# TurakhiaLab/TWILIGHT

Measured on AMD Instinct MI355X. Metric: DP band cells/s, TALCO-XDrop progressive profile-profile alignment (bit-exact vs reference CPU path), higher is better.
Workload: dtype f32

## Files before the change

### include/twl_align.h

```cpp
#ifndef TWL_ALIGN_H
#define TWL_ALIGN_H

#include <stdint.h>

#ifdef __cplusplus
extern "C" {
#endif

#define TWL_MAX_MATRIX 21
#define TWL_MAX_MARKER 1024

enum twl_status {
    TWL_OK = 0,
    TWL_ERR_NOT_INITIALIZED = -1,
    TWL_ERR_BAD_ARGUMENT = -2,
    TWL_ERR_HIP = -3,
    TWL_ERR_UNSUPPORTED = -4
};

typedef struct twl_params {
    int32_t P;
    float   matrix[TWL_MAX_MATRIX * TWL_MAX_MATRIX];
    float   gap_open;
    float   gap_extend;
// ... 43 lines not shown

int twl_copy_to_device(int device, void *dst_dev, const void *src, uint64_t bytes);
int twl_copy_from_device(int device, void *dst, const void *src_dev, uint64_t bytes);
int twl_copy_rows_from_device(int device, void *dst, uint64_t dst_pitch, const void *src_dev, uint64_t src_pitch, uint64_t width, uint64_t rows);

int twl_get_stats(int device, twl_stats *out);

int twl_get_pair_cells(int device, uint64_t *cells_out, int32_t n);

int twl_column_scores(const twl_params *p, int32_t seq_len, const float *freq, const int32_t *len, const int32_t *num, float *out);

int twl_dp_column_scores(const twl_params *p, int32_t seq_len, const float *freq, const float *gap_open, const float *gap_extend,
                         const int32_t *len, const int32_t *num, float *out);

#define TWL_MT_REC_WORDS 12
typedef struct twl_mt_dims {
    int32_t n_run, slots, sp_pitch, segcap;
    int32_t n_scout, n_tile, rounds;
    int32_t lead2, marg, anchors;
    int32_t thr, small_tiles, marker;
    int32_t reserved[3];
} twl_mt_dims;
int twl_mt_tables(int device, twl_mt_dims *dims, int32_t *order, int32_t *anchor, int32_t *spath, int32_t *chain, int32_t *rec, int8_t *seg, int32_t *front);

#define TWL_COMM_ID_BYTES 128
int twl_comm_unique_id(void *id128);
int twl_comm_init(int device, int rank, int world, const void *id128);
int twl_comm_all_gather(int device, const void *d_send, void *d_recv, int64_t bytes_per_rank);
int twl_comm_all_gather_host(int device, const void *send, void *recv, int64_t bytes_per_rank);
int twl_comm_destroy(int device);

enum twl_knob { TWL_KNOB_MT_PERTURB = 1, TWL_KNOB_MT_MAX_PAIRS = 2, TWL_KNOB_MT_MIN_MARKER = 3, TWL_KNOB_MT_LEAD = 4, TWL_KNOB_MT_MARGIN = 5,
                TWL_KNOB_MT_ROUNDS = 6, TWL_KNOB_MT_THR_JOBS = 7, TWL_KNOB_FAIL_ROW_ALLOCS = 8,
                TWL_KNOB_PROT_MODE = 9, TWL_KNOB_ASSUME_ONEHOT_QUERY = 10, TWL_KNOB_MT_TAIL_PCT = 11, TWL_KNOB_MT_WIDE = 12, TWL_KNOB_NO_SPEC = 13, TWL_KNOB_SCOUT_XDROP_PCT = 14, TWL_KNOB_THR_SMALL = 15, TWL_KNOB_FORCE_GLOBAL = 16, TWL_KNOB_LEAF_STEP = 17, TWL_KNOB_POISON_TB = 18, TWL_KNOB_MT_ANCHOR = 19, TWL_KNOB_MT_LEAD2 = 20, TWL_KNOB_PROT_CORRIDOR = 21 };
int twl_set_knob(int key, int value);
int twl_plan_describe(const twl_params *p, int32_t n_pairs, const int32_t *len, int32_t num_cu, int32_t qry_onehot, int32_t wide_streak, char *out, int32_t cap);

#ifdef __cplusplus
}
#endif
#endif
```

### twilight_amd/api.py

```python
from __future__ import annotations

import ctypes as C
import os

import numpy as np

_HERE = os.path.dirname(os.path.abspath(__file__))
LIB_PATH = os.environ.get("TWL_LIB") or os.path.join(_HERE, "libtwl_align.so")
TWL_MAX_MATRIX = 21

_lib = None


class TwlError(RuntimeError):
    pass


class TwlParams(C.Structure):
    _fields_ = [("P", C.c_int32), ("matrix", C.c_float * (TWL_MAX_MATRIX * TWL_MAX_MATRIX)), ("gap_open", C.c_float),
                ("gap_extend", C.c_float), ("gap_boundary", C.c_float), ("gap_char", C.c_float), ("xdrop", C.c_int32),
                ("flen", C.c_int32), ("marker", C.c_int32)]


class TwlStats(C.Structure):
# ... 94 lines not shown
    n, sl = batch.n_pairs, batch.seq_len
    freq = np.ascontiguousarray(batch.freq, dtype=np.float32)
    go = np.ascontiguousarray(batch.gap_open, dtype=np.float32)
    ge = np.ascontiguousarray(batch.gap_extend, dtype=np.float32)
    ln = np.ascontiguousarray(batch.len, dtype=np.int32)
    nm = np.ascontiguousarray(batch.num, dtype=np.int32)
    aln = np.zeros((n, 2 * sl), dtype=np.int8)
    aln_len = np.zeros(n, dtype=np.int32)
    err = np.zeros(n, dtype=np.int16)
    _check(lib.twl_align_batch(C.byref(params), C.c_int32(n), C.c_int32(sl), _ptr(freq, C.c_float), _ptr(go, C.c_float),
                               _ptr(ge, C.c_float), _ptr(ln, C.c_int32), _ptr(nm, C.c_int32), _ptr(aln, C.c_int8),
                               _ptr(aln_len, C.c_int32), _ptr(err, C.c_int16)))
    return aln, aln_len, err


def align_batch_device(params: TwlParams, n_pairs, seq_len, d_freq, d_gop, d_gex, d_len, d_num, d_aln, d_aln_len, d_err,
                       device=0, stream=None):
    lib = load_library()
    vp = C.c_void_p
    _check(lib.twl_align_batch_device(C.c_int(device), vp(stream or 0), C.byref(params), C.c_int32(n_pairs), C.c_int32(seq_len),
                                      vp(d_freq), vp(d_gop), vp(d_gex), vp(d_len), vp(d_num), vp(d_aln), vp(d_aln_len),
                                      vp(d_err)))


KNOB_MT_PERTURB, KNOB_MT_MAX_PAIRS, KNOB_MT_MIN_MARKER, KNOB_MT_LEAD, KNOB_MT_MARGIN, KNOB_MT_ROUNDS, KNOB_MT_THR_JOBS, KNOB_FAIL_ROW_ALLOCS = 1, 2, 3, 4, 5, 6, 7, 8
KNOB_PROT_MODE, KNOB_ASSUME_ONEHOT_QUERY, KNOB_MT_TAIL_PCT, KNOB_MT_WIDE, KNOB_NO_SPEC, KNOB_SCOUT_XDROP_PCT = 9, 10, 11, 12, 13, 14
KNOB_THR_SMALL = 15
KNOB_FORCE_GLOBAL = 16
KNOB_LEAF_STEP = 17
KNOB_POISON_TB = 18
KNOB_MT_ANCHOR = 19
KNOB_PROT_CORRIDOR = 21
KNOB_MT_LEAD2 = 20
PROT_MODES = {"auto": 0, "dense": 1, "sparse": 2, "presim": 3, "r1": 4, "lean_sparse": 5, "lean_presim": 6}


def set_knob(key: int, value: int):
    _check(load_library().twl_set_knob(C.c_int(key), C.c_int(value)))


def plan_describe(params, lens, num_cu=256, qry_onehot=False, wide_streak=0, small_state=0) -> str:
    wide_streak = int(wide_streak) + (100000 * (32 + int(small_state)) if small_state else 0)
    lens = np.ascontiguousarray(lens, dtype=np.int32)
    buf = C.create_string_buffer(256)
    _check(load_library().twl_plan_describe(C.byref(params), C.c_int32(lens.shape[0]), _ptr(lens, C.c_int32), C.c_int32(num_cu), C.c_int32(int(qry_onehot)), C.c_int32(wide_streak), buf, C.c_int32(256)))
    return buf.value.decode()


def version() -> str:
    return load_library().twl_version().decode()


def get_stats(device=0) -> TwlStats:
    st = TwlStats()
    _check(load_library().twl_get_stats(C.c_int(device), C.byref(st)))
    return st


def get_pair_cells(n, device=0):
    out = np.zeros(n, dtype=np.uint64)
    _check(load_library().twl_get_pair_cells(C.c_int(device), _ptr(out, C.c_uint64), C.c_int32(n)))
    return out


def column_scores(params: TwlParams, ref: np.ndarray, qry: np.ndarray, ref_num: int, qry_num: int) -> np.ndarray:
    ref = np.ascontiguousarray(ref, dtype=np.float32)
# ... 44 lines not shown
```

### twilight_amd/csrc/twl_align.hip

```cpp
#include "../../include/twl_align.h"
#include "../../include/twl_level.h"
#include "../../include/twl_place.h"
#include "../../include/twl_merge.h"
#include "../../include/twl_subtree.h"
#include "../../include/twl_guide.h"
#include "../../include/twl_retree.h"
#include "level_kernels.hip.h"
#include "restore_kernels.hip.h"
#include "place_kernels.hip.h"
#include "merge_kernels.hip.h"
#include "subtree_kernels.hip.h"
#include "guide_kernels.hip.h"
#include "retree_kernels.hip.h"
#include "talco_kernel.hip.h"
#include "talco_nuc.hip.h"
#include "talco_global.hip.h"

#include <hip/hip_runtime.h>
#include <dlfcn.h>

#include <algorithm>
#include <atomic>
#include <chrono>
#include <cmath>
// ... 46 lines not shown
#define HIP_TRY(expr)                                                                                          \
    do {                                                                                                       \
        hipError_t e_ = (expr);                                                                                \
        if (e_ != hipSuccess) {                                                                                \
            g_err = std::string(#expr) + ": " + hipGetErrorString(e_);                                         \
            return TWL_ERR_HIP;                                                                                \
        }                                                                                                      \
    } while (0)


#include "twl_policy.inc.hip"

struct Buf {
    void *p = nullptr;
    size_t cap = 0;
    int ensure(size_t bytes)
    {
        if (bytes <= cap) return TWL_OK;
        if (p) (void)hipFree(p);
        p = nullptr; cap = 0;
        size_t want = bytes + bytes / 8 + 256;
        HIP_TRY(hipMalloc(&p, want));
        cap = want;
        return TWL_OK;
    }
    void release() { if (p) (void)hipFree(p); p = nullptr; cap = 0; }
};

struct Device {
    int id = 0;
    hipStream_t stream = nullptr;
    hipStream_t stream2 = nullptr;
    hipEvent_t ev2[2] = {};
    hipEvent_t ev[8] = {};
    int num_cu = 0;
    Buf cols, tb, cells, queue, items, errs, dbg;
    Buf gtb;
    Buf sim, sim_off, blk_off, m24;
    Buf team;
    Buf mt_chain, mt_rec, mt_seg, mt_spath, mt_stat, mt_jobs, mt_anchor;
    Buf simdump;
    bool dump_on = false;
    std::vector<int32_t> dbg_host;
    std::vector<int32_t> mt_jobs_host;
    twl_mt_dims mt_dims{};
    std::vector<int32_t> mt_order;
    bool mt_seen = false;
    Buf gc_zero;
    std::vector<uint8_t> gc_zero_host;
    std::vector<int16_t> last_err;
    void *probe_h = nullptr; size_t probe_cap = 0;
    PassMemory mem;
    int live_stores = 0;
    void *comm = nullptr;
    int comm_world = 0, comm_rank = 0;
    Buf comm_send, comm_recv;
    int mt_launch = 0;
    char kname[160] = {0};
    Buf h2d_freq, h2d_gop, h2d_gex, h2d_len, h2d_num, d_aln, d_alnlen, d_err;
    twl_stats stats{};
    std::vector<uint64_t> pair_cells;
    twl::FillArgs fills{};
    char *res_h = nullptr; size_t res_cap = 0;
    std::vector<int32_t> last_alnlen;
    std::mutex mu;
};
// ... 46 lines not shown
}

static void twl_level_pool_release(Device *d);
namespace { extern int g_fail_next_row_allocs; void comm_destroy_raw(void *comm); }

extern "C" {

const char *twl_last_error(void) { return g_err.c_str(); }
#ifndef TWL_SOURCE_HASH
#define TWL_SOURCE_HASH "unstamped"
#endif
#ifndef TWL_BUILD_STAMP
#define TWL_BUILD_STAMP "unstamped"
#endif
__attribute__((used)) static const char twl_build_stamp[] = "TWLSTAMP:" TWL_BUILD_STAMP ";";
const char *twl_version(void) { return "twilight_amd 0.5 (gfx950) src " TWL_SOURCE_HASH; }

int twl_init(const int *device_ids, int n_devices)
{
    std::lock_guard<std::mutex> lk(g_mu);
    if (g_init) return TWL_OK;
    int count = 0;
    HIP_TRY(hipGetDeviceCount(&count));
    if (count < 1) { g_err = "no HIP device"; return TWL_ERR_HIP; }
    std::vector<int> ids;
    if (!device_ids || n_devices <= 0) ids.push_back(0);
    else ids.assign(device_ids, device_ids + n_devices);
    std::vector<Device *> devs;
    auto fail = [&](int rc) {
        for (auto *d : devs) {
            for (auto &e : d->ev) if (e) (void)hipEventDestroy(e);
            if (d->stream) (void)hipStreamDestroy(d->stream);
            if (d->stream2) (void)hipStreamDestroy(d->stream2);
            for (auto &e : d->ev2) if (e) (void)hipEventDestroy(e);
            delete d;
        }
        return rc;
    };
    for (int id : ids) {
        if (id < 0 || id >= count) { g_err = "device id out of range"; return fail(TWL_ERR_BAD_ARGUMENT); }
        auto *d = new Device();
        d->id = id;
        devs.push_back(d);
        hipDeviceProp_t prop;
        hipError_t e = hipSetDevice(id);
        if (e == hipSuccess) e = hipGetDeviceProperties(&prop, id);
        if (e == hipSuccess) { d->num_cu = prop.multiProcessorCount; e = hipStreamCreateWithFlags(&d->stream, hipStreamNonBlocking); if (e == hipSuccess) { int least = 0, greatest = 0; (void)hipDeviceGetStreamPriorityRange(&least, &greatest); e = hipStreamCreateWithPriority(&d->stream2, hipStreamNonBlocking, least); } }
        for (auto &ev : d->ev2) if (e == hipSuccess) e = hipEventCreate(&ev);
        for (auto &ev : d->ev) if (e == hipSuccess) e = hipEventCreate(&ev);
        if (e != hipSuccess) { g_err = std::string("twl_init: ") + hipGetErrorString(e); return fail(TWL_ERR_HIP); }
    }
    g_devs = devs;
    g_init = true;
#ifdef TWL_DEV
    static const struct { const char *env; int knob; } kEnvKnobs[] = {{"TWL_MT_MAX_PAIRS", TWL_KNOB_MT_MAX_PAIRS}, {"TWL_MT_LEAD", TWL_KNOB_MT_LEAD}, {"TWL_MT_MARGIN", TWL_KNOB_MT_MARGIN},
        {"TWL_MT_PERTURB", TWL_KNOB_MT_PERTURB}, {"TWL_MT_ROUNDS", TWL_KNOB_MT_ROUNDS}, {"TWL_MT_THR_JOBS", TWL_KNOB_MT_THR_JOBS}, {"TWL_MT_TAIL_PCT", TWL_KNOB_MT_TAIL_PCT}};
    for (const auto &k : kEnvKnobs) if (const char *v = getenv(k.env)) (void)twl_set_knob(k.knob, atoi(v));
#endif
    return TWL_OK;
}

void twl_shutdown(void)
{
    std::lock_guard<std::mutex> lk(g_mu);
    for (auto *d : g_devs) {
        std::lock_guard<std::mutex> dl(d->mu);
        if (d->live_stores > 0) {
            fprintf(stderr, "twl_shutdown: %d store(s) still alive on device %d; the library stays initialised (twl_store_destroy them first)\n", d->live_stores, d->id);
            return;
        }
    }
    for (auto *d : g_devs) {
        (void)hipSetDevice(d->id);
        (void)hipStreamSynchronize(d->stream);
        (void)hipStreamSynchronize(d->stream2);
        twl_level_pool_release(d);
        if (d->comm) { comm_destroy_raw(d->comm); d->comm = nullptr; }
        d->comm_send.release(); d->comm_recv.release();
        for (Buf *b : {&d->cols, &d->tb, &d->gtb, &d->cells, &d->queue, &d->items, &d->errs, &d->dbg, &d->sim, &d->sim_off, &d->blk_off, &d->m24, &d->team, &d->simdump, &d->mt_chain, &d->mt_rec, &d->mt_seg, &d->mt_spath, &d->mt_stat, &d->mt_jobs, &d->mt_anchor, &d->gc_zero,
                       &d->h2d_freq, &d->h2d_gop, &d->h2d_gex, &d->h2d_len, &d->h2d_num, &d->d_aln, &d->d_alnlen, &d->d_err})
            b->release();
        for (auto &e : d->ev) if (e) (void)hipEventDestroy(e);
        if (d->stream) (void)hipStreamDestroy(d->stream);
        if (d->stream2) (void)hipStreamDestroy(d->stream2);
        for (auto &e : d->ev2) if (e) (void)hipEventDestroy(e);
        if (d->res_h) (void)hipHostFree(d->res_h);
        if (d->probe_h) (void)hipHostFree(d->probe_h);
        delete d;
    }
    g_devs.clear();
    g_init = false;
}

int twl_align_batch_device(int device, void *stream, const twl_params *p, int32_t n_pairs, int32_t seq_len, const float *d_freq,
                           const float *d_gap_open, const float *d_gap_extend, const int32_t *d_len, const int32_t *d_num,
                           int8_t *d_aln_out, int32_t *d_aln_len_out, int16_t *d_err_out)
{
    if (!g_init) { g_err = "twl_init not called"; return TWL_ERR_NOT_INITIALIZED; }
    int rc = check_params(p);
    if (rc) return rc;
    if (n_pairs < 0 || seq_len < 1) { g_err = "bad n_pairs/seq_len"; return TWL_ERR_BAD_ARGUMENT; }
    Device *d = nullptr;
    if ((rc = find_dev(device, &d))) return rc;
    std::lock_guard<std::mutex> lk(d->mu);
    hipStream_t st = stream ? (hipStream_t)stream : d->stream;
    return run_device(d, st, p, n_pairs, seq_len, d_freq, d_gap_open, d_gap_extend, d_len, d_num, d_aln_out, d_aln_len_out,
                      d_err_out, nullptr);
}

static int run_host_slice(Device *d, const twl_params *p, const std::vector<int32_t> &ids, int32_t seq_len, const float *freq,
                          const float *gop, const float *gex, const int32_t *len, const int32_t *num, int8_t *aln_out,
                          int32_t *aln_len_out, int16_t *err_out)
{
    std::lock_guard<std::mutex> lk(d->mu);
    HIP_TRY(hipSetDevice(d->id));
    const int32_t n = (int32_t)ids.size();
    d->stats = twl_stats{};
    d->pair_cells.clear();
// ... 243 lines not shown
    int rc = find_dev(device, &d);
    if (rc) return rc;
    if (width == 0 || rows == 0) return TWL_OK;
    if (!dst || !src_dev || dst_pitch < width || src_pitch < width) { g_err = "bad argument"; return TWL_ERR_BAD_ARGUMENT; }
    HIP_TRY(hipSetDevice(d->id));
    HIP_TRY(hipMemcpy2D(dst, (size_t)dst_pitch, src_dev, (size_t)src_pitch, (size_t)width, (size_t)rows, hipMemcpyDeviceToHost));
    return TWL_OK;
}

int twl_set_knob(int key, int value)
{
    std::lock_guard<std::mutex> lk(g_mu);
    switch (key) {
    case TWL_KNOB_MT_PERTURB: g_mt_perturb = std::max(0, value); return TWL_OK;
    case TWL_KNOB_MT_MAX_PAIRS: g_mt_max_pairs = std::max(0, value); return TWL_OK;
    case TWL_KNOB_MT_MIN_MARKER: g_mt_min_marker = std::max(2, value); return TWL_OK;
    case TWL_KNOB_MT_LEAD: g_mt_lead = std::max(16, value); return TWL_OK;
    case TWL_KNOB_MT_MARGIN: if (value < 0) { g_mt_marg = 40; g_mt_marg_lat = 64; } else g_mt_marg = g_mt_marg_lat = std::max(2, value); return TWL_OK;
    case TWL_KNOB_MT_ROUNDS: g_mt_rounds = std::max(1, std::min(7, value)); return TWL_OK;
    case TWL_KNOB_MT_THR_JOBS: g_mt_thr_jobs = std::max(0, value); return TWL_OK;
    case TWL_KNOB_FAIL_ROW_ALLOCS: g_fail_next_row_allocs = std::max(0, value); return TWL_OK;
    case TWL_KNOB_PROT_MODE: if (value < 0 || value > 6) { g_err = "protein mode 0..6"; return TWL_ERR_BAD_ARGUMENT; } g_prot_mode = value; return TWL_OK;
    case TWL_KNOB_ASSUME_ONEHOT_QUERY: g_assume_onehot_query = value ? 1 : 0; return TWL_OK;
    case TWL_KNOB_MT_TAIL_PCT: g_mt_tail_pct = std::max(0, std::min(100, value)); return TWL_OK;
    case TWL_KNOB_MT_WIDE: g_mt_wide = value ? 1 : 0; return TWL_OK;
    case TWL_KNOB_NO_SPEC: g_no_spec = value ? 1 : 0; return TWL_OK;
    case TWL_KNOB_FORCE_GLOBAL: g_force_global = value ? 1 : 0; return TWL_OK;
    case TWL_KNOB_LEAF_STEP: g_leaf_step = value ? 1 : 0; return TWL_OK;
    case TWL_KNOB_POISON_TB: g_poison_tb = value ? 1 : 0; return TWL_OK;
    case TWL_KNOB_MT_ANCHOR: g_mt_anchor = value ? 1 : 0; return TWL_OK;
    case TWL_KNOB_MT_LEAD2: if (value < 0) { g_mt_lead2 = 96; g_mt_lead2_lat = 128; } else g_mt_lead2 = g_mt_lead2_lat = std::max(16, value); return TWL_OK;
    case TWL_KNOB_PROT_CORRIDOR: g_prot_corridor = std::max(0, value); for (auto *d : g_devs) d->mem.forget_corridor(); return TWL_OK;
    case TWL_KNOB_SCOUT_XDROP_PCT: g_scout_xdrop_pct = std::max(10, std::min(100, value)); return TWL_OK;
    case TWL_KNOB_THR_SMALL: g_thr_small = std::max(0, std::min(2, value)); for (auto *d : g_devs) d->mem.forget_small(); return TWL_OK;
    default: g_err = "unknown knob"; return TWL_ERR_BAD_ARGUMENT;
    }
}

#include "twl_comm.inc.hip"

int twl_plan_describe(const twl_params *p, int32_t n_pairs, const int32_t *len, int32_t num_cu, int32_t qry_onehot, int32_t wide_streak, char *out, int32_t cap)
{
    if (!p || (p->P != 6 && p->P != 22) || n_pairs < 0 || (n_pairs > 0 && !len) || num_cu < 1 || !out || cap < 64) { g_err = "bad argument (nucleotide or protein parameters, a buffer of 64+ bytes)"; return TWL_ERR_BAD_ARGUMENT; }
    const PassMemory mem = memory_from_code(wide_streak);
    std::vector<int32_t> order;
    for (int32_t n = 0; n < n_pairs; ++n) if (len[2 * n] > 0 && len[2 * n + 1] > 0) order.push_back(n);
    std::stable_sort(order.begin(), order.end(), [&](int32_t x, int32_t y) { return (int64_t)len[2 * x] + len[2 * x + 1] > (int64_t)len[2 * y] + len[2 * y + 1]; });
    const int ms = p->P - 1;
    std::vector<float> M(p->matrix, p->matrix + ms * ms);
    if (p->P == 22) {
        ProtFacts pf;
        pf.n_run = (int)order.size(); pf.n_pairs = n_pairs; pf.num_cu = num_cu; pf.marker = p->marker; pf.M = M.data(); pf.gap_char = p->gap_char;
        pf.corridor_lost = mem.corridor_lost; pf.h_len = len; pf.order = order.data();
        const ProtPlan pl = plan_protein(pf, current_knobs());
        const int w = snprintf(out, (size_t)cap, "%s; mode %d; window %d", prot_first_name(pl.first), pl.mm, prot_first_window(pl.first));
        if (pl.presim && w > 0 && w < cap) snprintf(out + w, (size_t)(cap - w), "; %zu scores precomputed, corridor %d", pl.simFloats, pl.corridor);
        return TWL_OK;
    }
    NucFacts nf;
    nf.n_run = (int)order.size(); nf.num_cu = num_cu; nf.marker = p->marker; nf.M = M.data(); nf.gap_char = p->gap_char; nf.qry_onehot = qry_onehot != 0;
    nf.remember(mem); nf.h_len = len; nf.order = order.data();
    const NucPlan pl = plan_nucleotide(nf, current_knobs());
    snprintf(out, (size_t)cap, "%s; mode %d; window %d%s; bulk %d tail %d", nuc_first_name(pl.first), pl.mm5 ? 5 : pl.mm,
             pl.first == NucFirst::WideMt ? 3072 : ((pl.first == NucFirst::Throughput && pl.small) ? 512 : ((pl.first == NucFirst::Throughput && pl.four) ? 768 : 1024)), pl.probe ? " or 768 (a sample of the level decides)" : "", pl.bulk, pl.tail);
    return TWL_OK;
}
// ... 34 lines not shown
```

### twilight_amd/csrc/twl_knobs.inc.hip

```cpp

int g_prot_corridor = 448;
int g_mt_perturb = 0;
int g_mt_lead = 320, g_mt_marg = 40;
int g_mt_marg_lat = 64, g_mt_lead2_lat = 128;
int g_mt_anchor = 1, g_mt_lead2 = 96;
int g_mt_max_pairs = 1024, g_mt_min_marker = 512, g_mt_rounds = 2, g_mt_thr_jobs = 256;
int g_scout_xdrop_pct = 100;
int g_no_spec = 0;
int g_thr_small = 0;
int g_mt_wide = 1;
int g_mt_tail_pct = 70;
int g_prot_mode = 0;
int g_force_global = 0;
int g_assume_onehot_query = 0;
int g_leaf_step = 1;
int g_poison_tb = 0;
Knobs current_knobs()
{
    return Knobs{g_mt_max_pairs, g_mt_min_marker, g_mt_tail_pct, g_mt_wide, g_assume_onehot_query, g_no_spec, g_thr_small, (ProtMode)g_prot_mode, g_prot_corridor,
                 g_mt_thr_jobs, g_mt_rounds, g_mt_anchor, g_mt_lead, g_mt_marg, g_mt_marg_lat, g_mt_lead2, g_mt_lead2_lat};
}
```

### twilight_amd/csrc/twl_launch.inc.hip

```cpp

template <class CfgT>
size_t tb_words_for(int marker) { return ((size_t)(marker >> 3) + 1) * (size_t)CfgT::WINDOW; }
int ensure_tb(Buf &b, hipStream_t st, size_t words, int grid)
{
    const size_t bytes = words * sizeof(uint32_t) * (size_t)grid;
    if (const int rc = b.ensure(bytes)) return rc;
    if (g_poison_tb) HIP_TRY(hipMemsetAsync(b.p, 0xFF, bytes, st));
    return TWL_OK;
}
template <auto Kernel, int THREADS>
int resident_per_cu(int *out)
{
    static std::atomic<int> cached{0};
    if (cached.load() == 0) {
        int nb = 0;
        HIP_TRY(hipOccupancyMaxActiveBlocksPerMultiprocessor(&nb, Kernel, THREADS, 0));
        cached.store(std::max(1, nb));
    }
    *out = cached.load();
    return TWL_OK;
}
twl::NArgs lean_args(const Device *d, const twl::KArgs &base)
{
    twl::NArgs a{};
// ... 82 lines not shown
}

template <int P, int W, int RPL, int MM, int MINW, bool SPEC = false, bool DUMP = false, int SP = 0>
int launch_lean(Device *d, hipStream_t st, const twl::KArgs &base, const int32_t *d_items, int n_items, int *grid_out, int *window_out)
{
    using CfgT = twl::NCfg<W, RPL>;
    int rc, blocks_per_cu = 0;
    if ((rc = resident_per_cu<twl::talco_lean_kernel<P, W, RPL, MM, MINW, SPEC, DUMP, 0, SP>, CfgT::THREADS>(&blocks_per_cu))) return rc;
    if (window_out) *window_out = CfgT::WINDOW;
    int grid = std::min(n_items, d->num_cu * blocks_per_cu);
    if (grid < 1) grid = 1;
    if (SPEC) {
        grid = 2 * n_items;
        if (grid > d->num_cu * blocks_per_cu) { g_err = "speculative launch larger than the device"; return TWL_ERR_BAD_ARGUMENT; }
    }
    const size_t tbw = tb_words_for<CfgT>(base.marker);
    if ((rc = ensure_tb(d->tb, st, tbw, grid))) return rc;
    twl::NArgs a = lean_args(d, base);
    a.tb = (uint32_t *)d->tb.p; a.tb_words = (int32_t)tbw; a.queue = base.queue; a.items = d_items; a.n_items = n_items; a.dbg = base.dbg;
    FILL_TRY(queue_fill(d, st, d->queue.p, sizeof(int32_t), 0));
    if (SPEC) {
        if ((rc = d->team.ensure((size_t)n_items * twl::kTeamWords * sizeof(unsigned long long)))) return rc;
        FILL_TRY(queue_fill(d, st, d->team.p, (size_t)n_items * twl::kTeamWords * sizeof(unsigned long long), 0));
        FILL_TRY(queue_fill(d, st, a.cells, (size_t)base.n_pairs_total * sizeof(unsigned long long), 0));
        a.team = (unsigned long long *)d->team.p;
    }
    TRACE("launch lean P=%d W=%d RPL=%d MM=%d grid=%d threads=%d n_items=%d tb_words=%zu", P, W, RPL, MM, grid, CfgT::THREADS, n_items, tbw);
    if (!d->kname[0]) {
        if constexpr (SP != 0) snprintf(d->kname, sizeof d->kname, "talco_lean_kernel<%d, %d, %d, %d, %d, %s, %s, 0, %d>", P, W, RPL, MM, MINW, SPEC ? "true" : "false", DUMP ? "true" : "false", SP);
        else snprintf(d->kname, sizeof d->kname, "talco_lean_kernel<%d, %d, %d, %d, %d, %s, %s, 0>", P, W, RPL, MM, MINW, SPEC ? "true" : "false", DUMP ? "true" : "false");
    }
    a.simdump = DUMP ? (float *)d->simdump.p : nullptr;
    FILL_TRY(flush_fills(d, st));
    hipLaunchKernelGGL((twl::talco_lean_kernel<P, W, RPL, MM, MINW, SPEC, DUMP, 0, SP>), dim3(grid), dim3(CfgT::THREADS), 0, st, a);
    HIP_TRY(hipGetLastError());
    if (SPEC && dbg_on()) {
        std::vector<unsigned long long> tw((size_t)n_items * twl::kTeamWords);
        HIP_TRY(hipMemcpyAsync(tw.data(), d->team.p, tw.size() * sizeof(unsigned long long), hipMemcpyDeviceToHost, st));
        HIP_TRY(hipStreamSynchronize(st));
        unsigned long long g = 0, h = 0;
        for (int t = 0; t < n_items; ++t) { g += tw[(size_t)t * twl::kTeamWords + twl::kTeamStat]; h += tw[(size_t)t * twl::kTeamWords + twl::kTeamStat + 1]; }
        fprintf(stderr, "[twl spec] %d pairs: %llu tile starts guessed, %llu confirmed\n", n_items, g, h);
    }
    *grid_out = grid;
    return TWL_OK;
}

template <int P, int W, int RPL, int MM, int MINW, int MT, int SP = 0>
int launch_mt_kernel(Device *d, hipStream_t st, twl::NArgs a, int n_items, int *grid_out = nullptr, size_t tb_groups = 0)
{
    using CfgT = twl::NCfg<W, RPL>;
    int rc, blocks_per_cu = 0;
    if ((rc = resident_per_cu<twl::talco_lean_kernel<P, W, RPL, MM, MINW, false, false, MT, SP>, CfgT::THREADS>(&blocks_per_cu))) return rc;
    int grid = std::max(1, std::min(n_items, d->num_cu * blocks_per_cu));
    const size_t tbw = tb_groups ? tb_groups * (size_t)CfgT::WINDOW : tb_words_for<CfgT>(a.marker);
    if (tb_groups) grid = (int)std::max<size_t>(1, std::min<size_t>((size_t)grid, ((size_t)8 << 30) / (tbw * sizeof(uint32_t))));
    if ((rc = ensure_tb(d->tb, st, tbw, grid))) return rc;
    a.tb = (uint32_t *)d->tb.p; a.tb_words = (int32_t)tbw; a.n_items = n_items;
    a.queue = (int32_t *)d->queue.p + (d->mt_launch++ % kMtCounters);
    FILL_TRY(flush_fills(d, st));
    hipLaunchKernelGGL((twl::talco_lean_kernel<P, W, RPL, MM, MINW, false, false, MT, SP>), dim3(grid), dim3(CfgT::THREADS), 0, st, a);
    HIP_TRY(hipGetLastError());
    if (grid_out) *grid_out = grid;
    return TWL_OK;
}


template <int W, int RPL, int MINW>
int launch_thr(Device *d, hipStream_t st, const twl::KArgs &a, const int32_t *items, int n, int *grid, int *window, bool mm5, int sp)
{
    if (mm5) {
        if (sp == 1) return launch_lean<6, W, RPL, 5, MINW, false, false, 1>(d, st, a, items, n, grid, window);
        return launch_lean<6, W, RPL, 5, MINW>(d, st, a, items, n, grid, window);
    }
    return launch_lean<6, W, RPL, 2, MINW>(d, st, a, items, n, grid, window);
}
template <int W, int RPL, int MM, int MINW, int MT>
int launch_mt_thr(Device *d, hipStream_t st, const twl::NArgs &a, int n_items, int *grid_out, int sp)
{
    if constexpr (MM == 5) { if (sp == 1) return launch_mt_kernel<6, W, RPL, MM, MINW, MT, 1>(d, st, a, n_items, grid_out); }
    return launch_mt_kernel<6, W, RPL, MM, MINW, MT>(d, st, a, n_items, grid_out);
}

int prepare_mt_tables(Device *d, hipStream_t st, const TilePlan &pl, const std::vector<int32_t> &jobs)
{
    int rc;
    if ((rc = d->mt_chain.ensure(pl.chain_ints * sizeof(int32_t)))) return rc;
    if ((rc = d->mt_rec.ensure(pl.rec_ints * sizeof(int32_t)))) return rc;
    if ((rc = d->mt_seg.ensure(pl.seg_bytes))) return rc;
    if ((rc = d->mt_spath.ensure(pl.spath_ints * sizeof(int32_t)))) return rc;
    if ((rc = d->mt_stat.ensure(pl.stat_bytes))) return rc;
    if ((rc = d->mt_jobs.ensure(pl.jobs_ints * sizeof(int32_t)))) return rc;
    if (pl.anchors && (rc = d->mt_anchor.ensure(pl.anchor_ints * sizeof(int32_t)))) return rc;
    HIP_TRY(hipMemcpyAsync(d->mt_jobs.p, jobs.data(), pl.jobs_ints * sizeof(int32_t), hipMemcpyHostToDevice, st));
    FILL_TRY(queue_fill(d, st, d->mt_rec.p, pl.rec_ints * sizeof(int32_t), 0));
    FILL_TRY(queue_fill(d, st, d->mt_spath.p, pl.spath_ints * sizeof(int32_t), 0xFE));
    FILL_TRY(queue_fill(d, st, d->mt_stat.p, pl.stat_bytes, 0));
    if (pl.anchors) FILL_TRY(queue_fill(d, st, d->mt_anchor.p, pl.anchor_ints * sizeof(int32_t), 0xFF));
    FILL_TRY(queue_fill(d, st, d->queue.p, kMtCounters * sizeof(int32_t), 0));
    d->mt_launch = 0;
    return TWL_OK;
}

static_assert(TWL_MT_REC_WORDS == twl::kMtRec, "include/twl_align.h states the words of a tile's record");
void remember_mt_plan(Device *d, const TilePlan &pl, const std::vector<int32_t> &order, int n_run, int marker)
{
    twl_mt_dims &m = d->mt_dims;
    m = twl_mt_dims{};
    m.n_run = n_run; m.slots = pl.slots; m.sp_pitch = pl.sp_pitch; m.segcap = pl.segcap; m.n_scout = pl.nScout; m.n_tile = pl.nTile; m.rounds = pl.rounds;
    m.lead2 = pl.lead2; m.marg = pl.marg; m.anchors = pl.anchors ? 1 : 0; m.thr = pl.thr ? 1 : 0; m.small_tiles = pl.smallT ? 1 : 0; m.marker = marker;
    d->mt_order.assign(order.begin(), order.begin() + n_run);
    d->mt_seen = true;
}
int read_mt_tables(Device *d, twl_mt_dims *dims, int32_t *order, int32_t *anchor, int32_t *spath, int32_t *chain, int32_t *rec, int8_t *seg, int32_t *front)
{
    if (!d->mt_seen) { g_err = "no tile-parallel level has run on this device since twl_init"; return TWL_ERR_BAD_ARGUMENT; }
    const twl_mt_dims &m = d->mt_dims;
    if (anchor && !m.anchors) { g_err = "the last tile-parallel level ran without anchors: there is no anchor table"; return TWL_ERR_BAD_ARGUMENT; }
    HIP_TRY(hipSetDevice(d->id));
    HIP_TRY(hipStreamSynchronize(d->stream));
    const size_t np = (size_t)m.n_run, ns = np * (size_t)m.slots;
    if (dims) *dims = m;
    if (order) std::copy(d->mt_order.begin(), d->mt_order.end(), order);
    if (np == 0) return TWL_OK;
    if (anchor) HIP_TRY(hipMemcpy(anchor, d->mt_anchor.p, ns * sizeof(int32_t), hipMemcpyDeviceToHost));
    if (spath) HIP_TRY(hipMemcpy(spath, d->mt_spath.p, np * (size_t)m.sp_pitch * sizeof(int32_t), hipMemcpyDeviceToHost));
    if (chain) HIP_TRY(hipMemcpy(chain, d->mt_chain.p, ns * 2 * sizeof(int32_t), hipMemcpyDeviceToHost));
    if (rec) HIP_TRY(hipMemcpy(rec, d->mt_rec.p, ns * twl::kMtRec * sizeof(int32_t), hipMemcpyDeviceToHost));
    if (seg) HIP_TRY(hipMemcpy(seg, d->mt_seg.p, ns * (size_t)m.segcap, hipMemcpyDeviceToHost));
    if (front) HIP_TRY(hipMemcpy(front, (const unsigned long long *)d->mt_stat.p + 4, np * 8 * sizeof(int32_t), hipMemcpyDeviceToHost));
    return TWL_OK;
}
// ... 65 lines not shown
```

### twilight_amd/csrc/twl_run.inc.hip

```cpp

struct Call {
    Device *d; hipStream_t st; const twl_params *p;
    int32_t n_pairs, seq_len;
    const int32_t *d_len, *d_num; int32_t *d_alnlen; int16_t *d_err;
    const int32_t *h_len;
    std::vector<int32_t> len_host, order;
    int32_t n_run = 0;
    uint64_t nominal = 0;
    twl::KArgs a{};
    const int32_t *items() const { return (const int32_t *)d->items.p; }
    long long len_sum(int32_t pr) const { return (long long)h_len[2 * pr] + h_len[2 * pr + 1]; }
};
struct Results { std::vector<int16_t> err; std::vector<unsigned long long> cells; unsigned long long mt[4] = {0, 0, 0, 0}; };

int pinned_at_least(void **h, size_t *cap, size_t bytes)
{
    if (bytes <= *cap) return TWL_OK;
    if (*h) (void)hipHostFree(*h);
    *h = nullptr; *cap = 0;
    HIP_TRY(hipHostMalloc(h, bytes + bytes / 2, hipHostMallocDefault));
    *cap = bytes + bytes / 2;
    return TWL_OK;
}

// ... 142 lines not shown
{
    Device *d = c.d; hipStream_t st = c.st; std::vector<int32_t> &order = c.order; const int bulk = pl.bulk;
    const int S = d->num_cu;
    std::vector<int32_t> front, rest;
    front.reserve((size_t)S); rest.reserve((size_t)bulk);
    for (int t = 0, nextPick = 0, j = 0; t < bulk; ++t) {
        if (j < S && t == nextPick) { front.push_back(order[t]); ++j; nextPick = (int)((long long)j * bulk / S); }
        else rest.push_back(order[t]);
    }
    std::copy(front.begin(), front.end(), order.begin());
    std::copy(rest.begin(), rest.end(), order.begin() + (std::ptrdiff_t)front.size());
    HIP_TRY(hipMemcpyAsync(d->items.p, order.data(), (size_t)bulk * sizeof(int32_t), hipMemcpyHostToDevice, st));
    *done = (int)front.size();
    FILL_TRY((launch_thr<4, 2, 5>(d, st, c.a, c.items(), *done, grid, window, pl.mm5, pl.sp)));
    FILL_TRY(pinned_at_least(&d->probe_h, &d->probe_cap, (size_t)c.n_pairs * sizeof(int16_t)));
    HIP_TRY(hipMemcpyAsync(d->probe_h, c.d_err, (size_t)c.n_pairs * sizeof(int16_t), hipMemcpyDeviceToHost, st));
    HIP_TRY(hipStreamSynchronize(st));
    int outgrew = 0;
    for (int32_t pr : front) outgrew += ((const int16_t *)d->probe_h)[pr] == twl::kErrOverflow ? 1 : 0;
    *small = outgrew * 100 <= 1 * *done;
    d->mem.small_state = *small ? 1 : -1;
    ran.probed = !*small;
    TRACE("sample of %d pairs on the 512-row window: %d outgrew it -> the level runs on %d rows", *done, outgrew, *small ? 512 : 768);
    d->kname[0] = 0;
    return TWL_OK;
}

int first_throughput(Call &c, const NucPlan &pl, Ran &ran, int *grid, int *window)
{
    Device *d = c.d; hipStream_t st = c.st; const int32_t *items = c.items(); const int bulk = pl.bulk, tail = pl.tail;
    bool small = pl.small;
    int done = 0, rc;
    if (pl.probe && bulk >= 8 * d->num_cu && (rc = sample_small_window(c, pl, ran, grid, window, &small, &done))) return rc;
    if (pl.four) rc = small ? launch_thr<4, 2, 5>(d, st, c.a, items + done, bulk - done, grid, window, pl.mm5, pl.sp)
                            : launch_thr<4, 3, 4>(d, st, c.a, items + done, bulk - done, grid, window, pl.mm5, pl.sp);
    else rc = with_mm<1, 0>(pl.mm, [&](auto MM) { return launch_lean<6, 8, 2, MM_OF(MM), 2>(d, st, c.a, items, bulk, grid, window); });
    ran.start = small ? Level::From512 : (pl.four ? Level::From768 : Level::Mid);
    if (rc || tail <= 0) return rc;
    const std::vector<int32_t> tailOrder(c.order.begin() + bulk, c.order.begin() + c.n_run);
    int g2 = 0, w2 = 0;
    ran.smallTiles = small && !ran.probed;
    ran.ranMt = true;
    return with_mm<5, 2>(ran.mode, [&](auto MM) { return launch_mt<6, MM_OF(MM), 3, false, 4>(d, st, c.a, items + bulk, tailOrder, tail, c.h_len, &g2, &w2, ran.smallTiles, pl.sp); });
}

int first_nucleotide(Call &c, bool qry_onehot, int shape, Ran &ran, int *grid, int *window)
{
    Device *d = c.d; hipStream_t st = c.st; const twl::KArgs &a = c.a; const int32_t *items = c.items(); const int32_t n_run = c.n_run;
    NucFacts nf;
    nf.n_run = n_run; nf.num_cu = d->num_cu; nf.marker = c.p->marker; nf.M = a.M; nf.gap_char = c.p->gap_char; nf.qry_onehot = qry_onehot; nf.shape = shape; nf.dump = d->dump_on;
    nf.remember(d->mem); nf.h_len = c.h_len; nf.order = c.order.data();
    const NucPlan pl = plan_nucleotide(nf, current_knobs());
    if (pl.first == NucFirst::Throughput && (pl.small || pl.held_back)) d->mem.begin_small_level(n_run);
    const int mode = pl.mm5 ? 5 : pl.mm;
    ran.mode = mode;
    ran.leanMid = pl.lean && pl.mm == 2;
    ran.start = Level::Mid;
    TRACE("plan: %s%s, matrix mode %d%s", nuc_first_name(pl.first), pl.small ? " (512-row window, five workgroups per CU)" : "", pl.mm, pl.mm5 ? " (one-letter query rows)" : "");
    switch (pl.first) {
    case NucFirst::Dump:
        if (!pl.lean || n_run != 1) { g_err = "score dump: one pair, matrix within the fast-division range"; return TWL_ERR_UNSUPPORTED; }
        return with_mm<5, 2, 1, 0>(mode, [&](auto MM) { return launch_lean<6, 16, 1, MM_OF(MM), 1, false, true>(d, st, a, items, n_run, grid, window); });
    case NucFirst::WideMt:
        ran.spec = 3; ran.ranMt = true; ran.startedWide = true; ran.start = Level::Wide;
        return launch_mt<6, 2, 3, true, 4>(d, st, a, items, c.order, n_run, c.h_len, grid, window);
    case NucFirst::Mt:
        ran.smallTiles = nf.small_state > 0;
        ran.spec = 3; ran.ranMt = true;
        return launch_mt<6, 2, 3, false, 4>(d, st, a, items, c.order, n_run, c.h_len, grid, window, ran.smallTiles, pl.sp);
    case NucFirst::SpecShared:
        ran.mode = 2; ran.spec = 2;
        return launch_lean<6, 8, 2, 2, 4, true>(d, st, a, items, n_run, grid, window);
    case NucFirst::Spec16:
        ran.spec = 1;
        return with_mm<5, 2>(mode, [&](auto MM) { return launch_lean<6, 16, 1, MM_OF(MM), 1, true>(d, st, a, items, n_run, grid, window); });
    case NucFirst::Few16:
// ... 95 lines not shown
    return TWL_OK;
}

int global_stage(Call &c, const Ran &ran, Results &res, bool anyMt, float *ms_redo)
{
    const std::vector<int32_t> redo = pairs_with(res.err, twl::kErrOverflow, twl::kErrGuard);
    int rc, w2 = 0;
    if (!redo.empty()) {
        if ((rc = timed_rerun(c, ran, Rung::Global, redo, ms_redo, &w2))) return rc;
        c.d->stats.window = std::max(c.d->stats.window, w2);
        if ((rc = collect(c, anyMt, res, true, nullptr))) return rc;
    }
    if (!pairs_with(res.err, twl::kErrOverflow, twl::kErrGuard).empty()) { g_err = "internal: a re-run code survived the global-memory kernel"; return TWL_ERR_HIP; }
    return TWL_OK;
}

int run_device(Device *d, hipStream_t st, const twl_params *p, int32_t n_pairs, int32_t seq_len, const float *d_freq,
               const float *d_gop, const float *d_gex, const int32_t *d_len, const int32_t *d_num, int8_t *d_aln,
               int32_t *d_alnlen, int16_t *d_err, const int32_t *h_len, const float *d_packed = nullptr, bool qry_onehot = false,
               const uint8_t *h_gc_zero = nullptr, int shape = 0)
{
    HIP_TRY(hipSetDevice(d->id));
    d->stats = twl_stats{};
    d->kname[0] = 0;
    d->fills.n = 0;
    d->last_err.clear();
    d->last_alnlen.clear();
    d->pair_cells.assign((size_t)n_pairs, 0);
    if (n_pairs == 0) return TWL_OK;

    int rc;
    if (!d_packed && (rc = d->cols.ensure((size_t)n_pairs * 2 * (size_t)seq_len * (size_t)(p->P + 2) * sizeof(float)))) return rc;
    if ((rc = d->cells.ensure((size_t)n_pairs * sizeof(unsigned long long)))) return rc;
    if ((rc = d->queue.ensure(64))) return rc;
    if ((rc = d->items.ensure((size_t)n_pairs * sizeof(int32_t)))) return rc;
    Call c{d, st, p, n_pairs, seq_len, d_len, d_num, d_alnlen, d_err, h_len};
    if ((rc = order_pairs(c))) return rc;
    if ((rc = prepare_args(c, d_freq, d_gop, d_gex, d_aln, d_packed, h_gc_zero))) return rc;

    Ran ran;
    ran.prot = (p->P == 22);
    ran.start = ran.prot ? Level::Wide : Level::Mid;
    int grid = 0, window = 0;
    if (c.n_run == 0) rc = TWL_OK;
    else if (g_force_global) {
        rc = ran.prot ? launch_global<22>(d, st, c.a, c.items(), c.n_run, seq_len, &grid, &window) : launch_global<6>(d, st, c.a, c.items(), c.n_run, seq_len, &grid, &window);
        snprintf(d->kname, sizeof d->kname, "talco_global_kernel<%d>", ran.prot ? 22 : 6);
    }
    else rc = ran.prot ? first_protein(c, ran, &grid, &window) : first_nucleotide(c, qry_onehot, shape, ran, &grid, &window);
    if (rc) return rc;
    FILL_TRY(flush_fills(d, st));
    HIP_TRY(hipEventRecord(d->ev[2], st));
    d->stats.n_launches = 1;
    d->stats.grid = grid;
    d->stats.window = window;
    d->stats.matrix_mode = ran.mode;
    d->stats.speculative = ran.spec;
    memcpy(d->stats.kernel, d->kname, sizeof d->stats.kernel);

    Results res;
    res.err.resize((size_t)n_pairs); res.cells.resize((size_t)n_pairs);
    LadderOutcome o;
    float ms_redo = 0.f;
    FILL_TRY(pinned_at_least((void **)&d->res_h, &d->res_cap, 4 * sizeof(unsigned long long) + (size_t)n_pairs * (sizeof(unsigned long long) + sizeof(int32_t) + sizeof(int16_t))));
    if ((rc = climb_ladder(c, ran, res, o, &ms_redo))) return rc;
    d->mem.update(ran, o, c.n_run, c.n_run > 0 ? c.len_sum(c.order[0]) : 0, current_knobs());
    if ((rc = global_stage(c, ran, res, ran.ranMt || o.redoMt, &ms_redo))) return rc;
// ... 26 lines not shown
```

Measured before the change: 233.7 billion.

## Run the level's multi-tile remainder on a side stream beside the bulk launch

Adds a low-priority tail stream, a separate traceback buffer and a separate set of work-queue counters, so the multi-tile remainder pairs can run concurrently with the bulk lean kernel instead of after it. An event is recorded just before the bulk launch; the tail stream waits on it, runs the MT kernel, then the main stream joins on a second event. This aims to fill GPU idle time while the bulk launch drains, at the cost of extra traceback memory, resource contention between the two kernels, and more complex synchronisation. It is enabled by default through a new knob.

```diff
diff --git a/include/twl_align.h b/include/twl_align.h
--- a/include/twl_align.h
+++ b/include/twl_align.h
@@ -99,7 +99,7 @@
 
 enum twl_knob { TWL_KNOB_MT_PERTURB = 1, TWL_KNOB_MT_MAX_PAIRS = 2, TWL_KNOB_MT_MIN_MARKER = 3, TWL_KNOB_MT_LEAD = 4, TWL_KNOB_MT_MARGIN = 5,
                 TWL_KNOB_MT_ROUNDS = 6, TWL_KNOB_MT_THR_JOBS = 7, TWL_KNOB_FAIL_ROW_ALLOCS = 8,
-                TWL_KNOB_PROT_MODE = 9, TWL_KNOB_ASSUME_ONEHOT_QUERY = 10, TWL_KNOB_MT_TAIL_PCT = 11, TWL_KNOB_MT_WIDE = 12, TWL_KNOB_NO_SPEC = 13, TWL_KNOB_SCOUT_XDROP_PCT = 14, TWL_KNOB_THR_SMALL = 15, TWL_KNOB_FORCE_GLOBAL = 16, TWL_KNOB_LEAF_STEP = 17, TWL_KNOB_POISON_TB = 18, TWL_KNOB_MT_ANCHOR = 19, TWL_KNOB_MT_LEAD2 = 20, TWL_KNOB_PROT_CORRIDOR = 21 };
+                TWL_KNOB_PROT_MODE = 9, TWL_KNOB_ASSUME_ONEHOT_QUERY = 10, TWL_KNOB_MT_TAIL_PCT = 11, TWL_KNOB_MT_WIDE = 12, TWL_KNOB_NO_SPEC = 13, TWL_KNOB_SCOUT_XDROP_PCT = 14, TWL_KNOB_THR_SMALL = 15, TWL_KNOB_FORCE_GLOBAL = 16, TWL_KNOB_LEAF_STEP = 17, TWL_KNOB_POISON_TB = 18, TWL_KNOB_MT_ANCHOR = 19, TWL_KNOB_MT_LEAD2 = 20, TWL_KNOB_PROT_CORRIDOR = 21, TWL_KNOB_TAIL_OVERLAP = 22 };
 int twl_set_knob(int key, int value);
 int twl_plan_describe(const twl_params *p, int32_t n_pairs, const int32_t *len, int32_t num_cu, int32_t qry_onehot, int32_t wide_streak, char *out, int32_t cap);
 
diff --git a/twilight_amd/api.py b/twilight_amd/api.py
--- a/twilight_amd/api.py
+++ b/twilight_amd/api.py
@@ -150,6 +150,7 @@
 KNOB_MT_ANCHOR = 19
 KNOB_PROT_CORRIDOR = 21
 KNOB_MT_LEAD2 = 20
+KNOB_TAIL_OVERLAP = 22
 PROT_MODES = {"auto": 0, "dense": 1, "sparse": 2, "presim": 3, "r1": 4, "lean_sparse": 5, "lean_presim": 6}
 
 
diff --git a/twilight_amd/csrc/twl_align.hip b/twilight_amd/csrc/twl_align.hip
--- a/twilight_amd/csrc/twl_align.hip
+++ b/twilight_amd/csrc/twl_align.hip
@@ -102,6 +102,11 @@
     hipStream_t stream = nullptr;
     hipStream_t stream2 = nullptr;
     hipEvent_t ev2[2] = {};
+    hipStream_t tail_stream = nullptr;
+    hipEvent_t tail_ev[2] = {};
+    Buf tb_tail;
+    bool tail_side = false;
+    bool fork_next = false;
     hipEvent_t ev[8] = {};
     int num_cu = 0;
     Buf cols, tb, cells, queue, items, errs, dbg;
@@ -214,7 +219,9 @@
             for (auto &e : d->ev) if (e) (void)hipEventDestroy(e);
             if (d->stream) (void)hipStreamDestroy(d->stream);
             if (d->stream2) (void)hipStreamDestroy(d->stream2);
+            if (d->tail_stream) (void)hipStreamDestroy(d->tail_stream);
             for (auto &e : d->ev2) if (e) (void)hipEventDestroy(e);
+            for (auto &e : d->tail_ev) if (e) (void)hipEventDestroy(e);
             delete d;
         }
         return rc;
@@ -227,8 +234,9 @@
         hipDeviceProp_t prop;
         hipError_t e = hipSetDevice(id);
         if (e == hipSuccess) e = hipGetDeviceProperties(&prop, id);
-        if (e == hipSuccess) { d->num_cu = prop.multiProcessorCount; e = hipStreamCreateWithFlags(&d->stream, hipStreamNonBlocking); if (e == hipSuccess) { int least = 0, greatest = 0; (void)hipDeviceGetStreamPriorityRange(&least, &greatest); e = hipStreamCreateWithPriority(&d->stream2, hipStreamNonBlocking, least); } }
+        if (e == hipSuccess) { d->num_cu = prop.multiProcessorCount; e = hipStreamCreateWithFlags(&d->stream, hipStreamNonBlocking); if (e == hipSuccess) { int least = 0, greatest = 0; (void)hipDeviceGetStreamPriorityRange(&least, &greatest); e = hipStreamCreateWithPriority(&d->stream2, hipStreamNonBlocking, least); if (e == hipSuccess) e = hipStreamCreateWithPriority(&d->tail_stream, hipStreamNonBlocking, least); } }
         for (auto &ev : d->ev2) if (e == hipSuccess) e = hipEventCreate(&ev);
+        for (auto &ev : d->tail_ev) if (e == hipSuccess) e = hipEventCreateWithFlags(&ev, hipEventDisableTiming);
         for (auto &ev : d->ev) if (e == hipSuccess) e = hipEventCreate(&ev);
         if (e != hipSuccess) { g_err = std::string("twl_init: ") + hipGetErrorString(e); return fail(TWL_ERR_HIP); }
     }
@@ -256,16 +264,19 @@
         (void)hipSetDevice(d->id);
         (void)hipStreamSynchronize(d->stream);
         (void)hipStreamSynchronize(d->stream2);
+        (void)hipStreamSynchronize(d->tail_stream);
         twl_level_pool_release(d);
         if (d->comm) { comm_destroy_raw(d->comm); d->comm = nullptr; }
         d->comm_send.release(); d->comm_recv.release();
-        for (Buf *b : {&d->cols, &d->tb, &d->gtb, &d->cells, &d->queue, &d->items, &d->errs, &d->dbg, &d->sim, &d->sim_off, &d->blk_off, &d->m24, &d->team, &d->simdump, &d->mt_chain, &d->mt_rec, &d->mt_seg, &d->mt_spath, &d->mt_stat, &d->mt_jobs, &d->mt_anchor, &d->gc_zero,
+        for (Buf *b : {&d->cols, &d->tb, &d->tb_tail, &d->gtb, &d->cells, &d->queue, &d->items, &d->errs, &d->dbg, &d->sim, &d->sim_off, &d->blk_off, &d->m24, &d->team, &d->simdump, &d->mt_chain, &d->mt_rec, &d->mt_seg, &d->mt_spath, &d->mt_stat, &d->mt_jobs, &d->mt_anchor, &d->gc_zero,
                        &d->h2d_freq, &d->h2d_gop, &d->h2d_gex, &d->h2d_len, &d->h2d_num, &d->d_aln, &d->d_alnlen, &d->d_err})
             b->release();
         for (auto &e : d->ev) if (e) (void)hipEventDestroy(e);
         if (d->stream) (void)hipStreamDestroy(d->stream);
         if (d->stream2) (void)hipStreamDestroy(d->stream2);
+        if (d->tail_stream) (void)hipStreamDestroy(d->tail_stream);
         for (auto &e : d->ev2) if (e) (void)hipEventDestroy(e);
+        for (auto &e : d->tail_ev) if (e) (void)hipEventDestroy(e);
         if (d->res_h) (void)hipHostFree(d->res_h);
         if (d->probe_h) (void)hipHostFree(d->probe_h);
         delete d;
@@ -575,6 +586,7 @@
     case TWL_KNOB_MT_LEAD2: if (value < 0) { g_mt_lead2 = 96; g_mt_lead2_lat = 128; } else g_mt_lead2 = g_mt_lead2_lat = std::max(16, value); return TWL_OK;
     case TWL_KNOB_PROT_CORRIDOR: g_prot_corridor = std::max(0, value); for (auto *d : g_devs) d->mem.forget_corridor(); return TWL_OK;
     case TWL_KNOB_SCOUT_XDROP_PCT: g_scout_xdrop_pct = std::max(10, std::min(100, value)); return TWL_OK;
+    case TWL_KNOB_TAIL_OVERLAP: g_tail_overlap = value ? 1 : 0; return TWL_OK;
     case TWL_KNOB_THR_SMALL: g_thr_small = std::max(0, std::min(2, value)); for (auto *d : g_devs) d->mem.forget_small(); return TWL_OK;
     default: g_err = "unknown knob"; return TWL_ERR_BAD_ARGUMENT;
     }
diff --git a/twilight_amd/csrc/twl_knobs.inc.hip b/twilight_amd/csrc/twl_knobs.inc.hip
--- a/twilight_amd/csrc/twl_knobs.inc.hip
+++ b/twilight_amd/csrc/twl_knobs.inc.hip
@@ -15,6 +15,7 @@
 int g_assume_onehot_query = 0;
 int g_leaf_step = 1;
 int g_poison_tb = 0;
+int g_tail_overlap = 1;
 Knobs current_knobs()
 {
     return Knobs{g_mt_max_pairs, g_mt_min_marker, g_mt_tail_pct, g_mt_wide, g_assume_onehot_query, g_no_spec, g_thr_small, (ProtMode)g_prot_mode, g_prot_corridor,
diff --git a/twilight_amd/csrc/twl_launch.inc.hip b/twilight_amd/csrc/twl_launch.inc.hip
--- a/twilight_amd/csrc/twl_launch.inc.hip
+++ b/twilight_amd/csrc/twl_launch.inc.hip
@@ -138,6 +138,7 @@
     }
     a.simdump = DUMP ? (float *)d->simdump.p : nullptr;
     FILL_TRY(flush_fills(d, st));
+    if (d->fork_next) { d->fork_next = false; HIP_TRY(hipEventRecord(d->tail_ev[0], st)); }
     hipLaunchKernelGGL((twl::talco_lean_kernel<P, W, RPL, MM, MINW, SPEC, DUMP, 0, SP>), dim3(grid), dim3(CfgT::THREADS), 0, st, a);
     HIP_TRY(hipGetLastError());
     if (SPEC && dbg_on()) {
@@ -152,6 +153,12 @@
     return TWL_OK;
 }
 
+constexpr int kTailCounterBase = 16;
+static_assert(kTailCounterBase >= kMtCounters && (kTailCounterBase * sizeof(int32_t)) % 16 == 0, "the remainder's counters start behind the level's, 16-byte aligned");
+constexpr size_t kQueueBytes = (size_t)(kTailCounterBase + kMtCounters) * sizeof(int32_t);
+Buf &mt_tb(Device *d) { return d->tail_side ? d->tb_tail : d->tb; }
+int32_t *mt_counters(Device *d) { return (int32_t *)d->queue.p + (d->tail_side ? kTailCounterBase : 0); }
+
 template <int P, int W, int RPL, int MM, int MINW, int MT, int SP = 0>
 int launch_mt_kernel(Device *d, hipStream_t st, twl::NArgs a, int n_items, int *grid_out = nullptr, size_t tb_groups = 0)
 {
@@ -159,11 +166,14 @@
     int rc, blocks_per_cu = 0;
     if ((rc = resident_per_cu<twl::talco_lean_kernel<P, W, RPL, MM, MINW, false, false, MT, SP>, CfgT::THREADS>(&blocks_per_cu))) return rc;
     int grid = std::max(1, std::min(n_items, d->num_cu * blocks_per_cu));
-    const size_t tbw = tb_groups ? tb_groups * (size_t)CfgT::WINDOW : tb_words_for<CfgT>(a.marker);
+    int tbMarker = a.marker;
+    if constexpr (MT == 2) tbMarker = std::max(tbMarker, std::min(a.mt_slots + 2 + a.mt_marg + std::max(a.mt_lead, a.mt_lead2), twl::kMaxMarker));
+    const size_t tbw = tb_groups ? tb_groups * (size_t)CfgT::WINDOW : tb_words_for<CfgT>(tbMarker);
     if (tb_groups) grid = (int)std::max<size_t>(1, std::min<size_t>((size_t)grid, ((size_t)8 << 30) / (tbw * sizeof(uint32_t))));
-    if ((rc = ensure_tb(d->tb, st, tbw, grid))) return rc;
-    a.tb = (uint32_t *)d->tb.p; a.tb_words = (int32_t)tbw; a.n_items = n_items;
-    a.queue = (int32_t *)d->queue.p + (d->mt_launch++ % kMtCounters);
+    Buf &tb = mt_tb(d);
+    if ((rc = ensure_tb(tb, st, tbw, grid))) return rc;
+    a.tb = (uint32_t *)tb.p; a.tb_words = (int32_t)tbw; a.n_items = n_items;
+    a.queue = mt_counters(d) + (d->mt_launch++ % kMtCounters);
     FILL_TRY(flush_fills(d, st));
     hipLaunchKernelGGL((twl::talco_lean_kernel<P, W, RPL, MM, MINW, false, false, MT, SP>), dim3(grid), dim3(CfgT::THREADS), 0, st, a);
     HIP_TRY(hipGetLastError());
@@ -203,7 +213,7 @@
     FILL_TRY(queue_fill(d, st, d->mt_spath.p, pl.spath_ints * sizeof(int32_t), 0xFE));
     FILL_TRY(queue_fill(d, st, d->mt_stat.p, pl.stat_bytes, 0));
     if (pl.anchors) FILL_TRY(queue_fill(d, st, d->mt_anchor.p, pl.anchor_ints * sizeof(int32_t), 0xFF));
-    FILL_TRY(queue_fill(d, st, d->queue.p, kMtCounters * sizeof(int32_t), 0));
+    FILL_TRY(queue_fill(d, st, mt_counters(d), kMtCounters * sizeof(int32_t), 0));
     d->mt_launch = 0;
     return TWL_OK;
 }
diff --git a/twilight_amd/csrc/twl_run.inc.hip b/twilight_amd/csrc/twl_run.inc.hip
--- a/twilight_amd/csrc/twl_run.inc.hip
+++ b/twilight_amd/csrc/twl_run.inc.hip
@@ -198,16 +198,32 @@
     bool small = pl.small;
     int done = 0, rc;
     if (pl.probe && bulk >= 8 * d->num_cu && (rc = sample_small_window(c, pl, ran, grid, window, &small, &done))) return rc;
+    const bool beside = tail > 0 && g_tail_overlap != 0;
+    d->fork_next = beside;
     if (pl.four) rc = small ? launch_thr<4, 2, 5>(d, st, c.a, items + done, bulk - done, grid, window, pl.mm5, pl.sp)
                             : launch_thr<4, 3, 4>(d, st, c.a, items + done, bulk - done, grid, window, pl.mm5, pl.sp);
     else rc = with_mm<1, 0>(pl.mm, [&](auto MM) { return launch_lean<6, 8, 2, MM_OF(MM), 2>(d, st, c.a, items, bulk, grid, window); });
     ran.start = small ? Level::From512 : (pl.four ? Level::From768 : Level::Mid);
+    const bool forked = beside && !d->fork_next;
+    d->fork_next = false;
     if (rc || tail <= 0) return rc;
     const std::vector<int32_t> tailOrder(c.order.begin() + bulk, c.order.begin() + c.n_run);
     int g2 = 0, w2 = 0;
     ran.smallTiles = small && !ran.probed;
     ran.ranMt = true;
-    return with_mm<5, 2>(ran.mode, [&](auto MM) { return launch_mt<6, MM_OF(MM), 3, false, 4>(d, st, c.a, items + bulk, tailOrder, tail, c.h_len, &g2, &w2, ran.smallTiles, pl.sp); });
+    hipStream_t ts = forked ? d->tail_stream : st;
+    if (forked) HIP_TRY(hipStreamWaitEvent(d->tail_stream, d->tail_ev[0], 0));
+    d->tail_side = forked;
+    rc = with_mm<5, 2>(ran.mode, [&](auto MM) { return launch_mt<6, MM_OF(MM), 3, false, 4>(d, ts, c.a, items + bulk, tailOrder, tail, c.h_len, &g2, &w2, ran.smallTiles, pl.sp); });
+    d->tail_side = false;
+    if (!forked) return rc;
+    if (!rc) rc = flush_fills(d, ts);
+    else d->fills.n = 0;
+    if (hipEventRecord(d->tail_ev[1], ts) != hipSuccess || hipStreamWaitEvent(st, d->tail_ev[1], 0) != hipSuccess) {
+        (void)hipStreamSynchronize(ts);
+        if (!rc) { g_err = "the join of a level's remainder with its bulk launch failed"; rc = TWL_ERR_HIP; }
+    }
+    return rc;
 }
 
 int first_nucleotide(Call &c, bool qry_onehot, int shape, Ran &ran, int *grid, int *window)
@@ -369,7 +385,7 @@
     int rc;
     if (!d_packed && (rc = d->cols.ensure((size_t)n_pairs * 2 * (size_t)seq_len * (size_t)(p->P + 2) * sizeof(float)))) return rc;
     if ((rc = d->cells.ensure((size_t)n_pairs * sizeof(unsigned long long)))) return rc;
-    if ((rc = d->queue.ensure(64))) return rc;
+    if ((rc = d->queue.ensure(kQueueBytes))) return rc;
     if ((rc = d->items.ensure((size_t)n_pairs * sizeof(int32_t)))) return rc;
     Call c{d, st, p, n_pairs, seq_len, d_len, d_num, d_alnlen, d_err, h_len};
     if ((rc = order_pairs(c))) return rc;
```

New measurement: 239.9 billion, median of 6. 2.7% higher.
